# 1879615351/Go-RIO

Hardware: AMD Instinct MI355X
Metric: APD-GICP GN iters/sec on 16k-pt scans + GP-preint windows/sec (higher is better)
Workload: dtype f32 search / f64 accumulate; 1 GPU; C4: 64 scan pairs 16384x16384 + 64 GP windows 1 s @ 200 Hz per GPU, k-NN covariances + 20 fixed GN iterations per pair; pairs_per_gpu=64, target_points=16384, optimizer=GN (convergence test disabled), search=pruned, parallelism=batch shard x1 (no collective)

## Files before the change

### go-rio_amd/csrc/ugpm_api.hip

```cpp
#include <hip/hip_runtime.h>

#include <algorithm>
#include <cmath>
#include <cstdlib>
#include <chrono>
#include <cstdio>
#include <cstring>
#include <limits>
#include <memory>
#include <string>
#include <atomic>
#include <vector>

#include "../../include/gorio_ugpm.h"
#include "ugpm_kernels.hip"
#include "ugpm_lpm_out.hip"
#include "ugpm_chunks.h"

using namespace gorio;

namespace {

#ifndef GORIO_EVAL_SPLIT
#define GORIO_EVAL_SPLIT 12
// ... 8 lines not shown
  int device = -1;
  hipStream_t stream = nullptr;
  hipStream_t stream2 = nullptr;
  hipEvent_t ev_jac = nullptr, ev_corr = nullptr, ev_up = nullptr;
  struct Group { hipStream_t s = nullptr, s2 = nullptr; hipEvent_t ev_jac = nullptr, ev_corr = nullptr, ev_done = nullptr, ev_tab = nullptr; };
  std::vector<Group> groups;
  double* ws = nullptr;
  size_t ws_cap = 0;
  UgpmWin* d_wins = nullptr;
  int wins_cap = 0;
  int* d_ints = nullptr;
  int lm_budget[2] = {0, 0};
  double* d_diag = nullptr;
  double* pin_in = nullptr;
  size_t pin_in_cap = 0;
  double* lpm_ws = nullptr;
  size_t lpm_ws_cap = 0;
  int* lpm_ints = nullptr;
  size_t lpm_ints_cap = 0;
  ug::LpmOutWin* d_lpm_wins = nullptr;
  int lpm_wins_cap = 0;
  std::vector<std::pair<hipEvent_t, hipEvent_t>> ev;
  std::vector<int> ev_stage;
};
thread_local Ctx g_ctx;
std::atomic<int> g_speculative_rot{1};

int ufail(int code, const std::string& msg) {
  g_err = msg;
  return code;
}

#define UHIP(expr)                                                                                              \
  do {                                                                                                          \
    hipError_t e_ = (expr);                                                                                     \
    if (e_ != hipSuccess) return ufail(GORIO_UGPM_ERR_NO_DEVICE, std::string(#expr) + ": " + hipGetErrorString(e_)); \
  } while (0)

struct HostWin {
  int g0 = 0, G = 0, v0 = 0, V = 0, S = 0;
  double state_freq = 0;
// ... 126 lines not shown
void gorio_ugpm_default_window(gorio_ugpm_window* w) {
  if (!w) return;
  std::memset(w, 0, sizeof(*w));
  w->type = GORIO_UGPM_TYPE_UGPM;
  w->min_freq = 500;
  w->quantum = -1;
  w->state_freq = 50.0;
  w->correlate = 1;
  w->overlap = 8;
  w->vel_bias_std = 0.3;
  w->gyr_bias_std = 0.03;
}

const char* gorio_ugpm_last_error(void) { return g_err.c_str(); }

void gorio_ugpm_debug_set_schedule(int speculative_rot) { g_speculative_rot.store(speculative_rot ? 1 : 0); }

int gorio_ugpm_get_stage_times(double seconds[8], int counts[8]) {
  for (int i = 0; i < 8; ++i) {
    if (seconds) seconds[i] = g_stage_s[i];
    if (counts) counts[i] = g_stage_n[i];
  }
  return 0;
}

static int preint_batch_flat(const gorio_ugpm_window* windows, int n_windows, gorio_ugpm_meas* out, gorio_ugpm_diag* diag, int device) {
  if (!windows || n_windows <= 0 || !out) return ufail(GORIO_UGPM_ERR_INVALID, "gorio_ugpm_preint_batch: bad arguments");
  int ndev = 0;
  if (hipGetDeviceCount(&ndev) != hipSuccess || ndev <= 0) return ufail(GORIO_UGPM_ERR_NO_DEVICE, "no usable HIP device (no CPU fallback exists)");
  if (device < 0 || device >= ndev) return ufail(GORIO_UGPM_ERR_INVALID, "bad device ordinal");
  UHIP(hipSetDevice(device));
  Ctx& c = g_ctx;
  if (c.device != device) {
    for (size_t g = 1; g < c.groups.size(); ++g) {
      hipStreamDestroy(c.groups[g].s); hipStreamDestroy(c.groups[g].s2);
      hipEventDestroy(c.groups[g].ev_jac); hipEventDestroy(c.groups[g].ev_corr);
    }
    for (auto& g : c.groups) { hipEventDestroy(g.ev_done); hipEventDestroy(g.ev_tab); }
    if (c.ev_up) hipEventDestroy(c.ev_up);
    if (c.stream) hipStreamDestroy(c.stream);
    if (c.stream2) hipStreamDestroy(c.stream2);
    if (c.ev_jac) hipEventDestroy(c.ev_jac);
    if (c.ev_corr) hipEventDestroy(c.ev_corr);
    hipFree(c.ws); hipFree(c.d_wins); hipFree(c.d_ints); hipFree(c.d_diag); hipFree(c.lpm_ws); hipFree(c.lpm_ints); hipFree(c.d_lpm_wins);
    if (c.pin_in) hipHostFree(c.pin_in);
    c = Ctx();
    c.device = device;
    bool made = false;
    if (!made) {
      int lo = 0, hi = 0;
      if (hipDeviceGetStreamPriorityRange(&lo, &hi) == hipSuccess && hipStreamCreateWithPriority(&c.stream, hipStreamNonBlocking, hi) == hipSuccess) made = true;
    }
    if (!made) UHIP(hipStreamCreateWithFlags(&c.stream, hipStreamNonBlocking));
    UHIP(hipStreamCreateWithFlags(&c.stream2, hipStreamNonBlocking));
    UHIP(hipEventCreateWithFlags(&c.ev_jac, hipEventDisableTiming));
    UHIP(hipEventCreateWithFlags(&c.ev_corr, hipEventDisableTiming));
    UHIP(hipFuncSetAttribute(reinterpret_cast<const void*>(&ug::corr_diag_kernel), hipFuncAttributeMaxDynamicSharedMemorySize, 140 * 1024));
    UHIP(hipFuncSetAttribute(reinterpret_cast<const void*>(&ug::infer_kernel), hipFuncAttributeMaxDynamicSharedMemorySize, 17 * (6 * 160 + 16) * 8) );
    {
      const void* fns[] = {reinterpret_cast<const void*>(&ug::ata_kernel<4, 16, kAtaTilesCorr>), reinterpret_cast<const void*>(&ug::ata_kernel<8, 16, kAtaTilesCorr>),
// ... 316 lines not shown
        ug::cross_kernel<<<dim3(12, r.nw, (std::max(max_G, max_V) + ug::kCrossRows - 1) / ug::kCrossRows), 256, sizeof(double) * ug::kCrossRows * (((max_S + 31) / 32) * 32 + 4), r.s>>>(dw_);
      }
      UHIP(hipEventRecord(r.ev_tab, r.s));
      UHIP(hipStreamWaitEvent(r.s2, r.ev_tab, 0));
      {
        Stage st(c, 2, r.s2);
        ug::corr_jac_kernel<<<dim3(ug::kCorrJacParts, r.nw), 256, 0, r.s2>>>(dw_);
        UHIP(hipEventRecord(r.ev_jac, r.s2));
        launch_ata(r, 2);
        ug::corr_factor_kernel<<<r.nw, 512, 0, r.s2>>>(dw_);
        ug::corr_diag_kernel<<<dim3((6 * max_S + 15) / 16, r.nw), 256, sizeof(double) * 17 * (6 * max_S + 16), r.s2>>>(dw_);
      }
      UHIP(hipEventRecord(r.ev_corr, r.s2));
    }
    std::vector<int> flags(kWinInts * (size_t)nw);
    const bool speculative = g_speculative_rot.load() != 0;
    for (int problem = 0; problem < 2; ++problem) {
      std::vector<std::unique_ptr<Stage>> st_lm;
      for (Run& r : runs) {
        const UgpmWin* dw_ = c.d_wins + r.g0;
        st_lm.emplace_back(new Stage(c, 3, r.s));
        ug::lm_begin_kernel<<<r.nw, 256, 0, r.s>>>(dw_, problem);
        if (problem == 0) ug::rot_eval_kernel<<<dim3(r.nw, kEvalSplit), 256, 0, r.s>>>(dw_, 2);
        else ug::vel_eval_kernel<<<dim3(r.nw, kEvalSplit), 256, 0, r.s>>>(dw_, 2);
        launch_ata(r, problem);
        r.active = true;
      }
      for (int it = 0; it <= 51; ++it) {
        bool any = false;
        for (Run& r : runs) {
          if (!r.active) continue;
          any = true;
          const UgpmWin* dw_ = c.d_wins + r.g0;
          ug::lm_step_kernel<<<dim3(r.nw, problem == 1 ? kVelBlocks : 1), 512, 0, r.s>>>(dw_);
          if (problem == 0 && speculative) {
            ug::rot_eval_kernel<<<dim3(r.nw, kEvalSplit), 256, 0, r.s>>>(dw_, 3);
            launch_ata(r, problem, 1);
            continue;
          }
          if (problem == 0) ug::rot_eval_kernel<<<dim3(r.nw, kEvalSplit), 256, 0, r.s>>>(dw_, 0);
          else ug::vel_eval_kernel<<<dim3(r.nw, kEvalSplit), 256, 0, r.s>>>(dw_, 0);
          if (problem == 0) {
            ug::rot_eval_kernel<<<dim3(r.nw, kEvalSplit), 256, 0, r.s>>>(dw_, 1);
// ... 45 lines not shown
    }
    for (Run& r : runs) {
      const UgpmWin* dw_ = c.d_wins + r.g0;
      UHIP(hipStreamWaitEvent(r.s, r.ev_corr, 0));
      {
        Stage st(c, 4, r.s);
        ug::finish_kernel<<<r.nw, 256, 0, r.s>>>(dw_);
        ug::infer_kernel<<<dim3(std::max(1, max_infer), r.nw), 256, sizeof(double) * 17 * (6 * max_S + 16), r.s>>>(dw_);
      }
      UHIP(hipEventRecord(r.ev_done, r.s));
    }
    for (size_t g = 1; g < runs.size(); ++g) UHIP(hipStreamWaitEvent(c.stream, runs[g].ev_done, 0));
    UHIP(hipGetLastError());
  }
  tt3 = tnow();
  std::vector<int> fin(kWinInts * (size_t)nw);
  std::vector<double> dg(4 * (size_t)nw);
  UHIP(hipMemcpyAsync(fin.data(), c.d_ints, sizeof(int) * fin.size(), hipMemcpyDeviceToHost, c.stream));
  UHIP(hipMemcpyAsync(dg.data(), c.d_diag, sizeof(double) * dg.size(), hipMemcpyDeviceToHost, c.stream));
  if (total_out) UHIP(hipMemcpyAsync(reinterpret_cast<double*>(out), out_region, sizeof(double) * total_out, hipMemcpyDeviceToHost, c.stream));
  UHIP(hipStreamSynchronize(c.stream));
  for (size_t q = 0; q < c.ev.size(); ++q) {
    float ms = 0.f;
    if (hipEventSynchronize(c.ev[q].second) == hipSuccess && hipEventElapsedTime(&ms, c.ev[q].first, c.ev[q].second) == hipSuccess) {
      g_stage_s[c.ev_stage[q]] += ms * 1e-3;
      g_stage_n[c.ev_stage[q]] += 1;
    }
    hipEventDestroy(c.ev[q].first);
    hipEventDestroy(c.ev[q].second);
  }
  c.ev.clear();
  c.ev_stage.clear();
  for (int i = 0; i < nw; ++i) {
    if (hw[i].status != 0) {
// ... 137 lines not shown
```

### go-rio_amd/csrc/ugpm_kernels.hip

```cpp
#include <hip/hip_runtime.h>
#include <math.h>

#include "ugpm_device.h"

namespace gorio {
namespace ug {

__device__ __forceinline__ UgpmWin load_win(const UgpmWin* __restrict__ wins, int i) {
  UgpmWin w;
  __builtin_memcpy(&w, (const __attribute__((address_space(4))) void*)(wins + i), sizeof(UgpmWin));
  return w;
}


#ifndef GORIO_UGPM_XCD
#define GORIO_UGPM_XCD 1
#endif
struct WinPart {
  int win, part, z;
};
__device__ __forceinline__ WinPart xcd_win_part() {
  WinPart r{(int)blockIdx.y, (int)blockIdx.x, (int)blockIdx.z};
#if GORIO_UGPM_XCD
  if (gridDim.y >= 16u && (gridDim.y & 7u) == 0u) {
// ... 1009 lines not shown
  }
}


__device__ __forceinline__ void small_gemm_tn_sym(const double* __restrict__ B, double* __restrict__ C, int S) {
  const int lane = threadIdx.x & 63, wave = threadIdx.x >> 6, nwave = (int)(blockDim.x >> 6);
  const int lr = lane & 15, lk = lane >> 4;
  const int T = (S + 15) / 16;
  for (int q = wave; q < T * (T + 1) / 2; q += nwave) {
    int tr = (int)((sqrtf(8.0f * (float)q + 1.0f) - 1.0f) * 0.5f);
    while (tr * (tr + 1) / 2 > q) --tr;
    while ((tr + 1) * (tr + 2) / 2 <= q) ++tr;
    const int tc = q - tr * (tr + 1) / 2;
    const int i = tr * 16 + lr, j = tc * 16 + lr;
    f64x4 acc = f64x4{0.0, 0.0, 0.0, 0.0};
#pragma unroll 4
    for (int k0 = tr * 16; k0 < S; k0 += 4) {
      const int k = k0 + lk;
      const double av = (k < S && i < S) ? B[(size_t)k * S + i] : 0.0;
      const double bv = (k < S && j < S) ? B[(size_t)k * S + j] : 0.0;
      acc = __builtin_amdgcn_mfma_f64_16x16x4f64(av, bv, acc, 0, 0, 0);
    }
#pragma unroll
    for (int rg = 0; rg < 4; ++rg) {
      const int r = tr * 16 + lk + 4 * rg, c = tc * 16 + lr;
      if (r < S && c < S) {
        C[(size_t)r * S + c] = acc[rg];
        C[(size_t)c * S + r] = acc[rg];
      }
    }
  }
}
__device__ __forceinline__ void small_gemm_nn(const double* __restrict__ A, const double* __restrict__ B, double* __restrict__ C, int S) {
  const int lane = threadIdx.x & 63, wave = threadIdx.x >> 6, nwave = (int)(blockDim.x >> 6);
  const int lr = lane & 15, lk = lane >> 4;
  const int T = (S + 15) / 16;
  for (int q = wave; q < T * T; q += nwave) {
    const int ti = q / T, tj = q - ti * T;
    const int i = ti * 16 + lr, j = tj * 16 + lr;
    f64x4 acc = f64x4{0.0, 0.0, 0.0, 0.0};
#pragma unroll 4
    for (int k0 = 0; k0 < S; k0 += 4) {
      const int k = k0 + lk;
      const double av = (k < S && i < S) ? A[(size_t)i * S + k] : 0.0;
      const double bv = (k < S && j < S) ? B[(size_t)k * S + j] : 0.0;
      acc = __builtin_amdgcn_mfma_f64_16x16x4f64(av, bv, acc, 0, 0, 0);
    }
#pragma unroll
    for (int rg = 0; rg < 4; ++rg) {
      const int r = ti * 16 + lk + 4 * rg, c = tj * 16 + lr;
      if (r < S && c < S) C[(size_t)r * S + c] = acc[rg];
    }
  }
}

__global__ __launch_bounds__(256) __attribute__((amdgpu_waves_per_eu(2, 2))) void gram_kernel(const UgpmWin* __restrict__ wins) {
// ... 88 lines not shown
  for (int r = wave; r < kCrossRows; r += 4) {
    const int n = row0 + r;
    for (int k = lane; k < LDK; k += 64) {
      double v = 0.0;
      if (n < N && k < S) v = integral ? se_kint(w.start_t, tt[n], w.state_t[k], l2, sf2) : se_k(tt[n], w.state_t[k], l2, sf2);
      ks[(size_t)r * LDK + k] = v;
    }
  }
  __syncthreads();
  const int lr = lane & 15, lk = lane >> 4;
  const int TJ = (S + 15) / 16;
  for (int q = wave; q < 2 * TJ; q += 4) {
    const int ti = q / TJ, tj = q - ti * TJ;
    const int j = tj * 16 + lr;
    f64x4 acc = f64x4{0.0, 0.0, 0.0, 0.0};
#pragma unroll 4
    for (int k0 = 0; k0 < S; k0 += 4) {
      const int k = k0 + lk;
      const double av = ks[(size_t)(ti * 16 + lr) * LDK + k];
      const double bv = (k < S && j < S) ? Ki[(size_t)k * S + j] : 0.0;
      acc = __builtin_amdgcn_mfma_f64_16x16x4f64(av, bv, acc, 0, 0, 0);
    }
#pragma unroll
    for (int rg = 0; rg < 4; ++rg) {
      const int n = row0 + ti * 16 + lk + 4 * rg;
      if (n < N && j < S) out[(size_t)n * S + j] = acc[rg];
    }
  }
}


// ... 73 lines not shown
  }
#pragma unroll
  for (int off = 32; off > 0; off >>= 1)
#pragma unroll
    for (int q = 0; q < 3; ++q) t[q] += __shfl_xor(t[q], off, 64);
#pragma unroll
  for (int q = 0; q < 3; ++q) out[q] = t[q];
}

__device__ __forceinline__ void lm_step_bookkeeping(const UgpmWin& w) {
  w.lmi[3] = 0;
  w.lmi[8] = 0;
  w.lmi[0] += 1;
}

__device__ int lm_decide_block(const UgpmWin& w, int m, int n, bool commit, double* sred ) {
  const int nblk = w.lmi[7] == 1 ? kVelBlocks : 1;
  bool step_ok = true;
  double mcc = 0.0, sn2 = 0.0;
  for (int q = 0; q < nblk; ++q) {
    step_ok = step_ok && w.lmi[9 + q] != 0;
    mcc += w.lmc[8 + q];
    sn2 += w.lmc[11 + q];
  }
  if (!(mcc > 0.0)) step_ok = false;
  const double sn = sqrt(sn2);
  if (!step_ok) {
    if (commit && threadIdx.x == 0) {
      w.lmc[2] = w.lmc[2] / w.lmc[3];
      w.lmc[3] *= 2.0;
// ... 14 lines not shown
  else if (fabs(cost_change) <= 1e-10 * cost) verdict = -1;
  else {
    rho = cost_change / mcc;
    verdict = rho > 1e-3 ? 1 : 0;
  }
  __syncthreads();
  if (commit) {
    if (threadIdx.x == 0) {
      w.lmc[1] = cost_new;
      if (verdict < 0) {
        w.lmi[1] = 1;
        w.lmi[5] = verdict == -2 ? 2 : 1;
      } else if (verdict == 1) {
        w.lmi[6] += 1;
        w.lmi[3] = 1;
        w.lmc[2] = fmin(1e16, w.lmc[2] / fmax(1.0 / 3.0, 1.0 - pow(2.0 * rho - 1.0, 3)));
        w.lmc[3] = 2.0;
        w.lmi[2] = 0;
      } else {
        w.lmc[2] = w.lmc[2] / w.lmc[3];
        w.lmc[3] *= 2.0;
        w.lmi[2] = 1;
      }
    }
    if (verdict == 1)
      for (int j = threadIdx.x; j < n; j += blockDim.x) w.lmv[5 * (size_t)n + j] = w.lmv[6 * (size_t)n + j];
  }
  return verdict < 0 ? -1 : verdict;
}

__device__ void gpnorm_rows(const UgpmWin& w, int ch, const double* __restrict__ s, double* __restrict__ res, double* __restrict__ J, int ldj, int col0, bool writeJ) {
  const int S = w.S;
  const double* KK = w.KKinv + (size_t)ch * S * S;
  const double* wt = w.wgp + (size_t)ch * S;
  if ((int)blockIdx.y != ch % (int)gridDim.y) return;
  for (int i = threadIdx.x; i < S; i += blockDim.x) res[i] = (row_dot(KK + (size_t)i * S, s, S) - s[i]) * wt[i];
  if (writeJ)
    for (int q = threadIdx.x; q < S * S; q += blockDim.x) {
      const int i = q / S, j = q % S;
      J[(size_t)i * ldj + col0 + j] = (KK[(size_t)j * S + i] - (i == j ? 1.0 : 0.0)) * wt[i];
    }
}

__global__ __launch_bounds__(256) void rot_eval_kernel(const UgpmWin* __restrict__ wins, int mode) {
  const UgpmWin w = load_win(wins, blockIdx.x);
  if (*w.status != 0 || w.lmi[1]) return;
  const int S = w.S, G = w.G, n = 3 * S;
  __shared__ double sred[8];
  if ((mode == 0 || mode == 3) && blockIdx.y == 0 && threadIdx.x == 0) lm_step_bookkeeping(w);
  if (mode == 1) {
    if (lm_decide_block(w, 3 * S + 3 * G, n, blockIdx.y == 0, sred) != 1) return;
  }
  const double* x = mode == 2 ? w.lmv + 5 * (size_t)n : w.lmv + 6 * (size_t)n;
  double* res = (mode == 0 || mode == 3) ? w.res_new : w.res;
  double* J = w.Jrot;
  const int i_lo = (int)(((long)G * blockIdx.y) / gridDim.y), i_hi = (int)(((long)G * (blockIdx.y + 1)) / gridDim.y);
// ... 52 lines not shown
        const double* k1 = w.KsKinv + ((size_t)c * G + i) * S;
        for (int j = lane; j < S; j += 64) row[c * S + j] = f0 * k0[j] + f1 * k1[j];
      }
    }
  }
}

__device__ __forceinline__ V3 vel_rot_vec(const UgpmWin& w, int i) {
  const int S = w.S, V = w.V;
  double rot[3];
  for (int c = 0; c < 3; ++c) rot[c] = row_dot(w.KgyrIntKinv + ((size_t)c * V + i) * S, w.s_dr + (size_t)c * S, S);
  const double dtm = w.vel_t[i] - w.start_t;
  return v3(rot[0] + dtm * w.hyper[3], rot[1] + dtm * w.hyper[7], rot[2] + dtm * w.hyper[11]);
}

__global__ __launch_bounds__(256) void vel_eval_kernel(const UgpmWin* __restrict__ wins, int mode) {
  const UgpmWin w = load_win(wins, blockIdx.x);
  if (*w.status != 0 || w.lmi[1]) return;
  if (mode == 1 && !w.lmi[3]) return;
  if (mode == 0 && blockIdx.y == 0 && threadIdx.x == 0) lm_step_bookkeeping(w);
  const int S = w.S, V = w.V, n = 3 * S;
  const double* x = mode == 0 ? w.lmv + 6 * (size_t)n : w.lmv + 5 * (size_t)n;
  double* res = mode == 0 ? w.res_new : w.res;
  double* J = w.Jvel;
  const int i_lo = (int)(((long)V * blockIdx.y) / gridDim.y), i_hi = (int)(((long)V * (blockIdx.y + 1)) / gridDim.y);
  if (mode == 2) {
    for (int c = 0; c < 3; ++c)
      if ((int)blockIdx.y == (3 + c) % (int)gridDim.y)
        for (size_t q = threadIdx.x; q < (size_t)S * n; q += blockDim.x) J[((size_t)3 * V + (size_t)c * S) * n + q] = 0.0;
    for (size_t q = threadIdx.x; q < (size_t)(i_hi - i_lo) * 3 * n; q += blockDim.x) J[(size_t)i_lo * 3 * n + q] = 0.0;
  }
  __syncthreads();
  for (int c = 0; c < 3; ++c) gpnorm_rows(w, 3 + c, x + (size_t)c * S, res + 3 * V + (size_t)c * S, J + ((size_t)3 * V + (size_t)c * S) * n, n, c * S, mode == 2);
  const double wgt = sqrt(1.0 / w.vel_var);
  __shared__ double sdot[256][6];
  for (int ib = i_lo; ib < i_hi; ib += 256) {
    const int cnt = min(256, i_hi - ib);
    for (int q = (int)(threadIdx.x >> 6); q < cnt; q += (int)(blockDim.x >> 6)) {
      const int i = ib + q;
      if (mode == 0) {
        double d3[3];
        wave_row_dots3(w.KvelKinv + (size_t)i * S, (size_t)V * S, x, S, d3);
        if ((threadIdx.x & 63) == 0) {
#pragma unroll
          for (int q2 = 0; q2 < 3; ++q2) sdot[q][3 + q2] = d3[q2];
        }
      } else {
        double d[6];
        wave_row_dots6(w.KgyrIntKinv + (size_t)i * S, (size_t)V * S, w.s_dr, w.KvelKinv + (size_t)i * S, (size_t)V * S, x, S, d);
        if ((threadIdx.x & 63) == 0) {
#pragma unroll
          for (int q2 = 0; q2 < 6; ++q2) sdot[q][q2] = d[q2];
        }
      }
    }
    __syncthreads();
    for (int q = threadIdx.x; q < cnt; q += blockDim.x) {
      const int i = ib + q;
      M3 RT;
      if (mode == 0) {
        RT = loadM(w.sample_tmp + (size_t)i * 24);
      } else {
        const double dtm = w.vel_t[i] - w.start_t;
        const V3 rv = v3(sdot[q][0] + dtm * w.hyper[3], sdot[q][1] + dtm * w.hyper[7], sdot[q][2] + dtm * w.hyper[11]);
        RT = expMap(v3(-rv.x, -rv.y, -rv.z));
      }
      const V3 vv = v3(sdot[q][3] + w.hyper[15], sdot[q][4] + w.hyper[19], sdot[q][5] + w.hyper[23]);
      const V3 t = mvec(RT, vv);
      double* r = res + 3 * i;
      r[0] = (t.x - (w.vel[i] - w.vel_bias[0])) * wgt;
      r[1] = (t.y - (w.vel[V + i] - w.vel_bias[1])) * wgt;
      r[2] = (t.z - (w.vel[2 * V + i] - w.vel_bias[2])) * wgt;
      if (mode != 0) storeM(w.sample_tmp + (size_t)i * 24, RT);
    }
    __syncthreads();
  }
  if (mode == 0) return;
  __syncthreads();
  {
    const int wave = threadIdx.x >> 6, lane = threadIdx.x & 63, nwave = (int)(blockDim.x >> 6);
    for (int rr = wave; rr < (i_hi - i_lo) * 3; rr += nwave) {
      const int i = i_lo + rr / 3, a = rr % 3;
      double* row = J + (size_t)(3 * i + a) * n;
      for (int c = 0; c < 3; ++c) {
        const double f = wgt * w.sample_tmp[(size_t)i * 24 + a * 3 + c];
        const double* k0 = w.KvelKinv + ((size_t)c * V + i) * S;
        for (int j = lane; j < S; j += 64) row[c * S + j] = f * k0[j];
      }
    }
  }
}
// ... 249 lines not shown
    }
    if (g != nullptr) {
      __syncthreads();
      if (gpart < gparts) ata_lds[gpart * gcolw + (int)threadIdx.x % gcolw] = gcol ? gacc : 0.0;
      __syncthreads();
      if (tid < gj1 - gj0) {
        double v = 0.0;
        for (int q = 0; q < gparts; ++q) v += ata_lds[q * gcolw + tid];
        g[gj0 + tid] = v;
      }
    }
  }
  CHOL_T(7);
}

__global__ __launch_bounds__(256) void lm_relinearize_linear_kernel(const UgpmWin* __restrict__ wins) {
  const UgpmWin w = load_win(wins, blockIdx.x);
  if (*w.status != 0 || w.lmi[1]) return;
  const int n = 3 * w.S, m = 3 * w.V + 3 * w.S;
  const int j0 = blockIdx.y * 64;
  if (j0 >= n) return;
  __shared__ double sred[8];
  if (lm_decide_block(w, m, n, blockIdx.y == 0, sred) != 1) return;
  const double* J = w.Jvel;
  const double* rn = w.res_new;
  __shared__ double sg[4][64];
  if (blockIdx.y == 0)
    for (int k = threadIdx.x; k < m; k += blockDim.x) w.res[k] = rn[k];
  const int slice = threadIdx.x >> 6, lane = threadIdx.x & 63;
  const int j = j0 + lane;
  double acc[4] = {0.0, 0.0, 0.0, 0.0};
  if (j < n) {
    int k = slice;
    for (; k + 12 < m; k += 16) {
#pragma unroll
      for (int u = 0; u < 4; ++u) acc[u] += J[(size_t)(k + 4 * u) * n + j] * rn[k + 4 * u];
    }
    for (; k < m; k += 4) acc[0] += J[(size_t)k * n + j] * rn[k];
  }
  sg[slice][lane] = (acc[0] + acc[1]) + (acc[2] + acc[3]);
  __syncthreads();
  if (slice == 0 && j < n) w.lmv[j] = (sg[0][lane] + sg[1][lane]) + (sg[2][lane] + sg[3][lane]);
}


__global__ __launch_bounds__(256) void lm_begin_kernel(const UgpmWin* __restrict__ wins, int problem) {
  const UgpmWin w = load_win(wins, blockIdx.x);
  if (*w.status != 0) return;
  const int n = 3 * w.S;
  const double* src = problem == 0 ? w.s_dr : w.s_vel;
  for (int j = threadIdx.x; j < n; j += blockDim.x) w.lmv[5 * (size_t)n + j] = src[j];
  if (threadIdx.x == 0) {
    for (int q = 0; q < 16; ++q) w.lmi[q] = 0;
    w.lmi[3] = 1;
    w.lmi[7] = problem;
    w.lmi[8] = 1;
    w.lmc[2] = 1e4;
    w.lmc[3] = 2.0;
  }
}

__global__ __launch_bounds__(512) void lm_step_kernel(const UgpmWin* __restrict__ wins) {
  const UgpmWin w = load_win(wins, blockIdx.x);
  if (*w.status != 0 || w.lmi[1]) return;
  const int n = 3 * w.S;
  const int problem = w.lmi[7];
  const int m = problem == 0 ? 3 * w.S + 3 * w.G : 3 * w.V + 3 * w.S;
  const int nblk = (int)gridDim.y, blk = (int)blockIdx.y;
  const int j0 = (int)((long)n * blk / nblk), j1 = (int)((long)n * (blk + 1) / nblk), ns = j1 - j0;
  double* g = w.lmv;
  double* scale = w.lmv + (size_t)n;
  double* diag = w.lmv + 2 * (size_t)n;
  double* step = w.lmv + 3 * (size_t)n;
  double* delta = w.lmv + 4 * (size_t)n;
  double* x = w.lmv + 5 * (size_t)n;
  double* xn = w.lmv + 6 * (size_t)n;
  __shared__ double sred[8];
  __shared__ int sflag;
  __shared__ CholLds chol;
  if (w.lmi[3]) {
    double c = 0.0;
    for (int k = threadIdx.x; k < m; k += blockDim.x) c += w.res[k] * w.res[k];
    c = 0.5 * block_sum(c, sred);
    double gm = 0.0, xn2 = 0.0;
    for (int j = threadIdx.x; j < n; j += blockDim.x) {
      gm = fmax(gm, fabs(g[j]));
      xn2 += x[j] * x[j];
    }
    gm = block_max(gm, sred);
    xn2 = block_sum(xn2, sred);
    if (w.lmi[8])
      for (int j = j0 + (int)threadIdx.x; j < j1; j += blockDim.x) scale[j] = 1.0 / (1.0 + sqrt(w.JtJ[(size_t)j * n + j]));
    __syncthreads();
    if (threadIdx.x == 0) {
      w.lmc[0] = c;
      w.lmc[4] = sqrt(xn2);
      if (w.lmi[8]) w.lmc[7] = c;
      if (gm <= 1e-10) {
        w.lmi[1] = 1;
        w.lmi[5] = 3;
      }
    }
    if (gm <= 1e-10) return;
  }
  if (w.lmi[0] >= 50) {
    if (threadIdx.x == 0) { w.lmi[1] = 1; w.lmi[5] = 4; }
    return;
  }
  const double radius = w.lmc[2];
  if (radius < 1e-32) {
    if (threadIdx.x == 0) { w.lmi[1] = 1; w.lmi[5] = 5; }
    return;
  }
  if (!w.lmi[2])
    for (int j = j0 + (int)threadIdx.x; j < j1; j += blockDim.x) diag[j] = fmin(fmax(w.JtJ[(size_t)j * n + j] * scale[j] * scale[j], 1e-6), 1e32);
  __syncthreads();
  double* L = w.lhs + (size_t)j0 * n + j0;
  __shared__ double xs[kCholMaxN / 2];
  const bool fused = ns < 384 && ns <= (int)blockDim.x && ns <= kCholMaxN / 2;
  for (int i = threadIdx.x >> 6; i < ns; i += (int)(blockDim.x >> 6)) {
    const double si = scale[j0 + i];
    for (int j = threadIdx.x & 63; j <= i; j += 64)
      L[(size_t)i * n + j] = w.JtJ[(size_t)(j0 + i) * n + j0 + j] * si * scale[j0 + j] + (i == j ? diag[j0 + i] / radius : 0.0);
  }
  double* rhs = w.lmv + 7 * (size_t)n + j0;
  for (int j = threadIdx.x; j < ns; j += blockDim.x) {
    step[j0 + j] = g[j0 + j] * scale[j0 + j];
    if (fused) rhs[j] = g[j0 + j] * scale[j0 + j];
  }
  __syncthreads();
  bool valid = block_cholesky(L, ns, n, chol, &sflag, fused ? rhs : nullptr);
  if (valid) {
    if (fused) {
      for (int j = threadIdx.x; j < ns; j += blockDim.x) xs[j] = rhs[j];
      __syncthreads();
      block_backward(L, ns, n, xs, chol);
      for (int j = threadIdx.x; j < ns; j += blockDim.x) step[j0 + j] = xs[j];
    } else {
      double* xp = &chol.P[0][0];
      for (int j = threadIdx.x; j < ns; j += blockDim.x) xp[j] = step[j0 + j];
      __syncthreads();
      if (threadIdx.x < 64) {
        wave_forward<1>(L, ns, n, xp, 1, 0);
        wave_backward(L, ns, n, xp);
      }
      __syncthreads();
// ... 16 lines not shown
      const double hi = 0.5 * delta[i];
      for (int j = j0 + (int)(threadIdx.x & 63); j < j1; j += 64) acc += hi * w.JtJ[(size_t)i * n + j] * delta[j];
    }
    for (int i = j0 + (int)threadIdx.x; i < j1; i += blockDim.x) {
      acc += delta[i] * g[i];
      sn2 += delta[i] * delta[i];
      xn[i] = x[i] + delta[i];
    }
    mcc = -block_sum(acc, sred);
    sn2 = block_sum(sn2, sred);
  }
  if (threadIdx.x == 0) {
    w.lmi[9 + blk] = valid ? 1 : 0;
    w.lmc[8 + blk] = mcc;
    w.lmc[11 + blk] = sn2;
  }
}


__global__ __launch_bounds__(256) void lm_end_kernel(const UgpmWin* __restrict__ wins, int problem, double* __restrict__ diag_out ) {
  const UgpmWin w = load_win(wins, blockIdx.x);
  if (*w.status != 0) return;
  const int n = 3 * w.S;
  double* dst = problem == 0 ? w.s_dr : w.s_vel;
  for (int j = threadIdx.x; j < n; j += blockDim.x) dst[j] = w.lmv[5 * (size_t)n + j];
  if (threadIdx.x == 0) {
    diag_out[blockIdx.x * 4 + problem * 2 + 0] = (double)w.lmi[0];
    diag_out[blockIdx.x * 4 + problem * 2 + 1] = w.lmc[0];
  }
}
// ... 273 lines not shown
```

### go-rio_amd/ugpm.py

```python
import ctypes as C

import numpy as np

from .apd import GorioError, load_library

LPM, UGPM = 0, 1
REC = 83

UGPM_SYMBOLS = ["gorio_ugpm_default_window", "gorio_ugpm_preint_batch", "gorio_ugpm_last_error", "gorio_ugpm_get_stage_times", "gorio_ugpm_debug_set_schedule",
                "gorio_ugpm_combine_preints"]


class UgpmWindow(C.Structure):

    _fields_ = [
        ("gyr_t", C.c_void_p), ("gyr", C.c_void_p), ("n_gyr", C.c_int),
        ("vel_t", C.c_void_p), ("vel", C.c_void_p), ("n_vel", C.c_int),
        ("gyr_var", C.c_double), ("vel_var", C.c_double), ("start_t", C.c_double),
        ("infer_t", C.c_void_p), ("n_infer", C.c_int), ("type", C.c_int),
        ("min_freq", C.c_double), ("quantum", C.c_double), ("state_freq", C.c_double),
        ("correlate", C.c_int), ("overlap", C.c_int),
        ("gyr_bias", C.c_double * 3), ("vel_bias", C.c_double * 3),
        ("vel_bias_std", C.c_double), ("gyr_bias_std", C.c_double),
        ("group_sizes", C.c_void_p), ("n_groups", C.c_int),
# ... 91 lines not shown
    return np.concatenate([np.asarray(m["delta_R"], np.float64).ravel(), np.asarray(m["delta_p"], np.float64), [m["dt"], m["dt_sq_half"]],
                           np.asarray(m["cov"], np.float64).ravel(), np.asarray(m["d_delta_R_d_bw"], np.float64).ravel(), np.asarray(m["d_delta_R_d_t"], np.float64),
                           np.asarray(m["d_delta_p_d_bw"], np.float64).ravel(), np.asarray(m["d_delta_p_d_bv"], np.float64).ravel(), np.asarray(m["d_delta_p_d_t"], np.float64)])


def ugpm_combine_preints(prev, cur):
    lib = load_library()
    a, b, out = np.ascontiguousarray(pack(prev)), np.ascontiguousarray(pack(cur)), np.zeros(REC)
    lib.gorio_ugpm_combine_preints.argtypes = [C.c_void_p, C.c_void_p, C.c_void_p]
    rc = lib.gorio_ugpm_combine_preints(C.c_void_p(_dp(a)), C.c_void_p(_dp(b)), C.c_void_p(_dp(out)))
    if rc < 0:
        raise GorioError(rc, lib.gorio_ugpm_last_error().decode())
    return unpack(out)


def ugpm_debug_set_schedule(speculative_rot=True):
    lib = load_library()
    lib.gorio_ugpm_debug_set_schedule.argtypes = [C.c_int]
    lib.gorio_ugpm_debug_set_schedule.restype = None
    lib.gorio_ugpm_debug_set_schedule(1 if speculative_rot else 0)


def ugpm_stage_times():
    lib = load_library()
    s = (C.c_double * 8)()
    c = (C.c_int * 8)()
    lib.gorio_ugpm_get_stage_times(s, c)
    return list(s), list(c)


class PreintOption:

    def __init__(self, min_freq=500.0, type=UGPM, quantum=-1.0, state_freq=50.0, correlate=True):
        self.min_freq, self.type, self.quantum, self.state_freq, self.correlate = min_freq, type, quantum, state_freq, correlate

# ... 59 lines not shown
```

### include/gorio_ugpm.h

```cpp
#ifndef GORIO_UGPM_H
#define GORIO_UGPM_H

#ifdef __cplusplus
extern "C" {
#endif

typedef enum {
  GORIO_UGPM_OK = 0,
  GORIO_UGPM_ERR_INVALID = -1,
  GORIO_UGPM_ERR_NO_DEVICE = -2,
  GORIO_UGPM_ERR_RANGE = -3,
  GORIO_UGPM_ERR_ARGUMENT = -4,
  GORIO_UGPM_ERR_UNSUPPORTED = -5,
  GORIO_UGPM_ERR_NUMERIC = -6
} gorio_ugpm_status;

typedef enum { GORIO_UGPM_TYPE_LPM = 0, GORIO_UGPM_TYPE_UGPM = 1 } gorio_ugpm_type;

typedef struct {
  const double* gyr_t;
  const double* gyr;
  int n_gyr;
  const double* vel_t;
  const double* vel;
// ... 40 lines not shown
  double cost_rot;
  double cost_vel;
  double state_freq;
} gorio_ugpm_diag;

void gorio_ugpm_default_window(gorio_ugpm_window* w);

int gorio_ugpm_preint_batch(const gorio_ugpm_window* windows, int n_windows, gorio_ugpm_meas* out, gorio_ugpm_diag* diag, int device);

int gorio_ugpm_combine_preints(const gorio_ugpm_meas* prev, const gorio_ugpm_meas* cur, gorio_ugpm_meas* out);

const char* gorio_ugpm_last_error(void);

int gorio_ugpm_get_stage_times(double seconds[8], int counts[8]);

void gorio_ugpm_debug_set_schedule(int speculative_rot);

#ifdef __cplusplus
}
#endif
#endif
```

Measured before the change: 164,500 linearisations/s.

## Fuse velocity LM solve into a single persistent per-window kernel launch

Adds vel_fit_kernel, which runs the whole velocity-problem Levenberg-Marquardt loop (step, residual evaluation, decision, gradient update) inside one launch per run. It replaces up to 52 host-driven passes of separate kernel launches and is the default schedule. The step, residual and gradient code is factored into shared device helpers. Output readback moves to a reusable pinned host buffer, and several GEMM loops change from unroll 4 to unroll 1, presumably to relieve register pressure. The risk is that one block per window serialises work that was previously split across kVelBlocks blocks, and that aliasing shared memory between the Cholesky panel and the scratch arrays needs careful synchronisation.

Result: slower. 142,300 linearisations/s (-13.5%).

```diff
diff --git a/go-rio_amd/csrc/ugpm_api.hip b/go-rio_amd/csrc/ugpm_api.hip
--- a/go-rio_amd/csrc/ugpm_api.hip
+++ b/go-rio_amd/csrc/ugpm_api.hip
@@ -46,6 +46,8 @@
   double* d_diag = nullptr;
   double* pin_in = nullptr;
   size_t pin_in_cap = 0;
+  char* pin_out = nullptr;
+  size_t pin_out_cap = 0;
   double* lpm_ws = nullptr;
   size_t lpm_ws_cap = 0;
   int* lpm_ints = nullptr;
@@ -56,7 +58,8 @@
   std::vector<int> ev_stage;
 };
 thread_local Ctx g_ctx;
-std::atomic<int> g_speculative_rot{1};
+std::atomic<int> g_schedule{1};
+constexpr int kLmMaxPasses = 52;
 
 int ufail(int code, const std::string& msg) {
   g_err = msg;
@@ -213,7 +216,7 @@
 
 const char* gorio_ugpm_last_error(void) { return g_err.c_str(); }
 
-void gorio_ugpm_debug_set_schedule(int speculative_rot) { g_speculative_rot.store(speculative_rot ? 1 : 0); }
+void gorio_ugpm_debug_set_schedule(int schedule) { g_schedule.store(schedule & 3); }
 
 int gorio_ugpm_get_stage_times(double seconds[8], int counts[8]) {
   for (int i = 0; i < 8; ++i) {
@@ -243,6 +246,7 @@
     if (c.ev_corr) hipEventDestroy(c.ev_corr);
     hipFree(c.ws); hipFree(c.d_wins); hipFree(c.d_ints); hipFree(c.d_diag); hipFree(c.lpm_ws); hipFree(c.lpm_ints); hipFree(c.d_lpm_wins);
     if (c.pin_in) hipHostFree(c.pin_in);
+    if (c.pin_out) hipHostFree(c.pin_out);
     c = Ctx();
     c.device = device;
     bool made = false;
@@ -589,7 +593,9 @@
       UHIP(hipEventRecord(r.ev_corr, r.s2));
     }
     std::vector<int> flags(kWinInts * (size_t)nw);
-    const bool speculative = g_speculative_rot.load() != 0;
+    const int schedule = g_schedule.load();
+    const bool speculative = (schedule & 1) != 0;
+    const bool fused_vel = (schedule & 2) == 0;
     for (int problem = 0; problem < 2; ++problem) {
       std::vector<std::unique_ptr<Stage>> st_lm;
       for (Run& r : runs) {
@@ -601,7 +607,23 @@
         launch_ata(r, problem);
         r.active = true;
       }
-      for (int it = 0; it <= 51; ++it) {
+      if (problem == 1 && fused_vel) {
+        for (size_t g = 0; g < runs.size(); ++g) {
+          ug::vel_fit_kernel<<<runs[g].nw, 512, 0, runs[g].s>>>(c.d_wins + runs[g].g0, kLmMaxPasses, c.d_diag + 4 * (size_t)runs[g].g0);
+          st_lm[g].reset();
+        }
+        if (lmtrace) {
+          double lc[16];
+          int li[16];
+          UHIP(hipStreamSynchronize(runs[0].s));
+          UHIP(hipMemcpy(lc, dw[0].lmc, sizeof(lc), hipMemcpyDeviceToHost));
+          UHIP(hipMemcpy(li, dw[0].lmi, sizeof(li), hipMemcpyDeviceToHost));
+          std::fprintf(stderr, "[ugpm lm] problem 1 (one launch): iter %d done %d term %d succ %d cost %.17g cost_new %.17g radius %.6g x_norm %.17g initial %.17g\n",
+                       li[0], li[1], li[5], li[6], lc[0], lc[1], lc[2], lc[4], lc[7]);
+        }
+        continue;
+      }
+      for (int it = 0; it < kLmMaxPasses; ++it) {
         bool any = false;
         for (Run& r : runs) {
           if (!r.active) continue;
@@ -677,10 +699,18 @@
     UHIP(hipGetLastError());
   }
   tt3 = tnow();
-  std::vector<int> fin(kWinInts * (size_t)nw);
-  std::vector<double> dg(4 * (size_t)nw);
-  UHIP(hipMemcpyAsync(fin.data(), c.d_ints, sizeof(int) * fin.size(), hipMemcpyDeviceToHost, c.stream));
-  UHIP(hipMemcpyAsync(dg.data(), c.d_diag, sizeof(double) * dg.size(), hipMemcpyDeviceToHost, c.stream));
+  const size_t dg_bytes = sizeof(double) * 4 * (size_t)nw, fin_bytes = sizeof(int) * kWinInts * (size_t)nw;
+  if (dg_bytes + fin_bytes > c.pin_out_cap) {
+    if (c.pin_out) hipHostFree(c.pin_out);
+    c.pin_out = nullptr;
+    c.pin_out_cap = 0;
+    UHIP(hipHostMalloc(reinterpret_cast<void**>(&c.pin_out), 2 * (dg_bytes + fin_bytes), hipHostMallocDefault));
+    c.pin_out_cap = 2 * (dg_bytes + fin_bytes);
+  }
+  const double* const dg = reinterpret_cast<const double*>(c.pin_out);
+  const int* const fin = reinterpret_cast<const int*>(c.pin_out + dg_bytes);
+  UHIP(hipMemcpyAsync(c.pin_out + dg_bytes, c.d_ints, fin_bytes, hipMemcpyDeviceToHost, c.stream));
+  UHIP(hipMemcpyAsync(c.pin_out, c.d_diag, dg_bytes, hipMemcpyDeviceToHost, c.stream));
   if (total_out) UHIP(hipMemcpyAsync(reinterpret_cast<double*>(out), out_region, sizeof(double) * total_out, hipMemcpyDeviceToHost, c.stream));
   UHIP(hipStreamSynchronize(c.stream));
   for (size_t q = 0; q < c.ev.size(); ++q) {
diff --git a/go-rio_amd/csrc/ugpm_kernels.hip b/go-rio_amd/csrc/ugpm_kernels.hip
--- a/go-rio_amd/csrc/ugpm_kernels.hip
+++ b/go-rio_amd/csrc/ugpm_kernels.hip
@@ -1047,7 +1047,7 @@
     const int tc = q - tr * (tr + 1) / 2;
     const int i = tr * 16 + lr, j = tc * 16 + lr;
     f64x4 acc = f64x4{0.0, 0.0, 0.0, 0.0};
-#pragma unroll 4
+#pragma unroll 1
     for (int k0 = tr * 16; k0 < S; k0 += 4) {
       const int k = k0 + lk;
       const double av = (k < S && i < S) ? B[(size_t)k * S + i] : 0.0;
@@ -1072,7 +1072,7 @@
     const int ti = q / T, tj = q - ti * T;
     const int i = ti * 16 + lr, j = tj * 16 + lr;
     f64x4 acc = f64x4{0.0, 0.0, 0.0, 0.0};
-#pragma unroll 4
+#pragma unroll 1
     for (int k0 = 0; k0 < S; k0 += 4) {
       const int k = k0 + lk;
       const double av = (k < S && i < S) ? A[(size_t)i * S + k] : 0.0;
@@ -1191,7 +1191,7 @@
     const int ti = q / TJ, tj = q - ti * TJ;
     const int j = tj * 16 + lr;
     f64x4 acc = f64x4{0.0, 0.0, 0.0, 0.0};
-#pragma unroll 4
+#pragma unroll 1
     for (int k0 = 0; k0 < S; k0 += 4) {
       const int k = k0 + lk;
       const double av = ks[(size_t)(ti * 16 + lr) * LDK + k];
@@ -1295,6 +1295,8 @@
   w.lmi[0] += 1;
 }
 
+__device__ __noinline__ double lm_cube(double v) { return pow(v, 3); }
+
 __device__ int lm_decide_block(const UgpmWin& w, int m, int n, bool commit, double* sred ) {
   const int nblk = w.lmi[7] == 1 ? kVelBlocks : 1;
   bool step_ok = true;
@@ -1339,7 +1341,7 @@
       } else if (verdict == 1) {
         w.lmi[6] += 1;
         w.lmi[3] = 1;
-        w.lmc[2] = fmin(1e16, w.lmc[2] / fmax(1.0 / 3.0, 1.0 - pow(2.0 * rho - 1.0, 3)));
+        w.lmc[2] = fmin(1e16, w.lmc[2] / fmax(1.0 / 3.0, 1.0 - lm_cube(2.0 * rho - 1.0)));
         w.lmc[3] = 2.0;
         w.lmi[2] = 0;
       } else {
@@ -1354,17 +1356,20 @@
   return verdict < 0 ? -1 : verdict;
 }
 
-__device__ void gpnorm_rows(const UgpmWin& w, int ch, const double* __restrict__ s, double* __restrict__ res, double* __restrict__ J, int ldj, int col0, bool writeJ) {
+__device__ void gpnorm_rows_block(const UgpmWin& w, int ch, const double* __restrict__ s, double* __restrict__ res, double* __restrict__ J, int ldj, int col0, bool writeJ) {
   const int S = w.S;
   const double* KK = w.KKinv + (size_t)ch * S * S;
   const double* wt = w.wgp + (size_t)ch * S;
-  if ((int)blockIdx.y != ch % (int)gridDim.y) return;
   for (int i = threadIdx.x; i < S; i += blockDim.x) res[i] = (row_dot(KK + (size_t)i * S, s, S) - s[i]) * wt[i];
   if (writeJ)
     for (int q = threadIdx.x; q < S * S; q += blockDim.x) {
       const int i = q / S, j = q % S;
       J[(size_t)i * ldj + col0 + j] = (KK[(size_t)j * S + i] - (i == j ? 1.0 : 0.0)) * wt[i];
     }
+}
+__device__ void gpnorm_rows(const UgpmWin& w, int ch, const double* __restrict__ s, double* __restrict__ res, double* __restrict__ J, int ldj, int col0, bool writeJ) {
+  if ((int)blockIdx.y != ch % (int)gridDim.y) return;
+  gpnorm_rows_block(w, ch, s, res, J, ldj, col0, writeJ);
 }
 
 __global__ __launch_bounds__(256) void rot_eval_kernel(const UgpmWin* __restrict__ wins, int mode) {
@@ -1447,6 +1452,52 @@
   return v3(rot[0] + dtm * w.hyper[3], rot[1] + dtm * w.hyper[7], rot[2] + dtm * w.hyper[11]);
 }
 
+__device__ __forceinline__ void vel_residual_rows(const UgpmWin& w, int mode, const double* __restrict__ x, double* __restrict__ res, int i_lo, int i_hi, double (*sdot)[6]) {
+  const int S = w.S, V = w.V;
+  const double wgt = sqrt(1.0 / w.vel_var);
+  for (int ib = i_lo; ib < i_hi; ib += 256) {
+    const int cnt = min(256, i_hi - ib);
+    for (int q = (int)(threadIdx.x >> 6); q < cnt; q += (int)(blockDim.x >> 6)) {
+      const int i = ib + q;
+      if (mode == 0) {
+        double d3[3];
+        wave_row_dots3(w.KvelKinv + (size_t)i * S, (size_t)V * S, x, S, d3);
+        if ((threadIdx.x & 63) == 0) {
+#pragma unroll
+          for (int q2 = 0; q2 < 3; ++q2) sdot[q][3 + q2] = d3[q2];
+        }
+      } else {
+        double d[6];
+        wave_row_dots6(w.KgyrIntKinv + (size_t)i * S, (size_t)V * S, w.s_dr, w.KvelKinv + (size_t)i * S, (size_t)V * S, x, S, d);
+        if ((threadIdx.x & 63) == 0) {
+#pragma unroll
+          for (int q2 = 0; q2 < 6; ++q2) sdot[q][q2] = d[q2];
+        }
+      }
+    }
+    __syncthreads();
+    for (int q = threadIdx.x; q < cnt; q += blockDim.x) {
+      const int i = ib + q;
+      M3 RT;
+      if (mode == 0) {
+        RT = loadM(w.sample_tmp + (size_t)i * 24);
+      } else {
+        const double dtm = w.vel_t[i] - w.start_t;
+        const V3 rv = v3(sdot[q][0] + dtm * w.hyper[3], sdot[q][1] + dtm * w.hyper[7], sdot[q][2] + dtm * w.hyper[11]);
+        RT = expMap(v3(-rv.x, -rv.y, -rv.z));
+      }
+      const V3 vv = v3(sdot[q][3] + w.hyper[15], sdot[q][4] + w.hyper[19], sdot[q][5] + w.hyper[23]);
+      const V3 t = mvec(RT, vv);
+      double* r = res + 3 * i;
+      r[0] = (t.x - (w.vel[i] - w.vel_bias[0])) * wgt;
+      r[1] = (t.y - (w.vel[V + i] - w.vel_bias[1])) * wgt;
+      r[2] = (t.z - (w.vel[2 * V + i] - w.vel_bias[2])) * wgt;
+      if (mode != 0) storeM(w.sample_tmp + (size_t)i * 24, RT);
+    }
+    __syncthreads();
+  }
+}
+
 __global__ __launch_bounds__(256) void vel_eval_kernel(const UgpmWin* __restrict__ wins, int mode) {
   const UgpmWin w = load_win(wins, blockIdx.x);
   if (*w.status != 0 || w.lmi[1]) return;
@@ -1467,47 +1518,7 @@
   for (int c = 0; c < 3; ++c) gpnorm_rows(w, 3 + c, x + (size_t)c * S, res + 3 * V + (size_t)c * S, J + ((size_t)3 * V + (size_t)c * S) * n, n, c * S, mode == 2);
   const double wgt = sqrt(1.0 / w.vel_var);
   __shared__ double sdot[256][6];
-  for (int ib = i_lo; ib < i_hi; ib += 256) {
-    const int cnt = min(256, i_hi - ib);
-    for (int q = (int)(threadIdx.x >> 6); q < cnt; q += (int)(blockDim.x >> 6)) {
-      const int i = ib + q;
-      if (mode == 0) {
-        double d3[3];
-        wave_row_dots3(w.KvelKinv + (size_t)i * S, (size_t)V * S, x, S, d3);
-        if ((threadIdx.x & 63) == 0) {
-#pragma unroll
-          for (int q2 = 0; q2 < 3; ++q2) sdot[q][3 + q2] = d3[q2];
-        }
-      } else {
-        double d[6];
-        wave_row_dots6(w.KgyrIntKinv + (size_t)i * S, (size_t)V * S, w.s_dr, w.KvelKinv + (size_t)i * S, (size_t)V * S, x, S, d);
-        if ((threadIdx.x & 63) == 0) {
-#pragma unroll
-          for (int q2 = 0; q2 < 6; ++q2) sdot[q][q2] = d[q2];
-        }
-      }
-    }
-    __syncthreads();
-    for (int q = threadIdx.x; q < cnt; q += blockDim.x) {
-      const int i = ib + q;
-      M3 RT;
-      if (mode == 0) {
-        RT = loadM(w.sample_tmp + (size_t)i * 24);
-      } else {
-        const double dtm = w.vel_t[i] - w.start_t;
-        const V3 rv = v3(sdot[q][0] + dtm * w.hyper[3], sdot[q][1] + dtm * w.hyper[7], sdot[q][2] + dtm * w.hyper[11]);
-        RT = expMap(v3(-rv.x, -rv.y, -rv.z));
-      }
-      const V3 vv = v3(sdot[q][3] + w.hyper[15], sdot[q][4] + w.hyper[19], sdot[q][5] + w.hyper[23]);
-      const V3 t = mvec(RT, vv);
-      double* r = res + 3 * i;
-      r[0] = (t.x - (w.vel[i] - w.vel_bias[0])) * wgt;
-      r[1] = (t.y - (w.vel[V + i] - w.vel_bias[1])) * wgt;
-      r[2] = (t.z - (w.vel[2 * V + i] - w.vel_bias[2])) * wgt;
-      if (mode != 0) storeM(w.sample_tmp + (size_t)i * 24, RT);
-    }
-    __syncthreads();
-  }
+  vel_residual_rows(w, mode, x, res, i_lo, i_hi, sdot);
   if (mode == 0) return;
   __syncthreads();
   {
@@ -1787,6 +1798,20 @@
   CHOL_T(7);
 }
 
+__device__ __forceinline__ double linear_gradient_slice(const double* __restrict__ J, const double* __restrict__ rn, int n, int m, int j, int slice) {
+  double acc[4] = {0.0, 0.0, 0.0, 0.0};
+  if (j < n) {
+    int k = slice;
+#pragma unroll 2
+    for (; k + 12 < m; k += 16) {
+#pragma unroll
+      for (int u = 0; u < 4; ++u) acc[u] += J[(size_t)(k + 4 * u) * n + j] * rn[k + 4 * u];
+    }
+    for (; k < m; k += 4) acc[0] += J[(size_t)k * n + j] * rn[k];
+  }
+  return (acc[0] + acc[1]) + (acc[2] + acc[3]);
+}
+
 __global__ __launch_bounds__(256) void lm_relinearize_linear_kernel(const UgpmWin* __restrict__ wins) {
   const UgpmWin w = load_win(wins, blockIdx.x);
   if (*w.status != 0 || w.lmi[1]) return;
@@ -1802,16 +1827,7 @@
     for (int k = threadIdx.x; k < m; k += blockDim.x) w.res[k] = rn[k];
   const int slice = threadIdx.x >> 6, lane = threadIdx.x & 63;
   const int j = j0 + lane;
-  double acc[4] = {0.0, 0.0, 0.0, 0.0};
-  if (j < n) {
-    int k = slice;
-    for (; k + 12 < m; k += 16) {
-#pragma unroll
-      for (int u = 0; u < 4; ++u) acc[u] += J[(size_t)(k + 4 * u) * n + j] * rn[k + 4 * u];
-    }
-    for (; k < m; k += 4) acc[0] += J[(size_t)k * n + j] * rn[k];
-  }
-  sg[slice][lane] = (acc[0] + acc[1]) + (acc[2] + acc[3]);
+  sg[slice][lane] = linear_gradient_slice(J, rn, n, m, j, slice);
   __syncthreads();
   if (slice == 0 && j < n) w.lmv[j] = (sg[0][lane] + sg[1][lane]) + (sg[2][lane] + sg[3][lane]);
 }
@@ -1833,24 +1849,18 @@
   }
 }
 
-__global__ __launch_bounds__(512) void lm_step_kernel(const UgpmWin* __restrict__ wins) {
-  const UgpmWin w = load_win(wins, blockIdx.x);
-  if (*w.status != 0 || w.lmi[1]) return;
-  const int n = 3 * w.S;
-  const int problem = w.lmi[7];
-  const int m = problem == 0 ? 3 * w.S + 3 * w.G : 3 * w.V + 3 * w.S;
-  const int nblk = (int)gridDim.y, blk = (int)blockIdx.y;
-  const int j0 = (int)((long)n * blk / nblk), j1 = (int)((long)n * (blk + 1) / nblk), ns = j1 - j0;
+struct LmStepLds {
+  double sred[8];
+  int sflag;
+  CholLds chol;
+  double xs[kCholMaxN / 2];
+};
+
+__device__ __forceinline__ bool lm_step_head(const UgpmWin& w, int n, int m, int j0, int j1, LmStepLds& sh) {
   double* g = w.lmv;
   double* scale = w.lmv + (size_t)n;
-  double* diag = w.lmv + 2 * (size_t)n;
-  double* step = w.lmv + 3 * (size_t)n;
-  double* delta = w.lmv + 4 * (size_t)n;
   double* x = w.lmv + 5 * (size_t)n;
-  double* xn = w.lmv + 6 * (size_t)n;
-  __shared__ double sred[8];
-  __shared__ int sflag;
-  __shared__ CholLds chol;
+  double* sred = sh.sred;
   if (w.lmi[3]) {
     double c = 0.0;
     for (int k = threadIdx.x; k < m; k += blockDim.x) c += w.res[k] * w.res[k];
@@ -1874,22 +1884,36 @@
         w.lmi[5] = 3;
       }
     }
-    if (gm <= 1e-10) return;
+    if (gm <= 1e-10) return false;
   }
   if (w.lmi[0] >= 50) {
     if (threadIdx.x == 0) { w.lmi[1] = 1; w.lmi[5] = 4; }
-    return;
-  }
+    return false;
+  }
+  if (w.lmc[2] < 1e-32) {
+    if (threadIdx.x == 0) { w.lmi[1] = 1; w.lmi[5] = 5; }
+    return false;
+  }
+  return true;
+}
+
+__device__ __forceinline__ void lm_step_block(const UgpmWin& w, int n, int j0, int j1, int blk, LmStepLds& sh) {
+  const int ns = j1 - j0;
+  double* g = w.lmv;
+  double* scale = w.lmv + (size_t)n;
+  double* diag = w.lmv + 2 * (size_t)n;
+  double* step = w.lmv + 3 * (size_t)n;
+  double* delta = w.lmv + 4 * (size_t)n;
+  double* x = w.lmv + 5 * (size_t)n;
+  double* xn = w.lmv + 6 * (size_t)n;
+  double* sred = sh.sred;
+  CholLds& chol = sh.chol;
+  double* xs = sh.xs;
   const double radius = w.lmc[2];
-  if (radius < 1e-32) {
-    if (threadIdx.x == 0) { w.lmi[1] = 1; w.lmi[5] = 5; }
-    return;
-  }
   if (!w.lmi[2])
     for (int j = j0 + (int)threadIdx.x; j < j1; j += blockDim.x) diag[j] = fmin(fmax(w.JtJ[(size_t)j * n + j] * scale[j] * scale[j], 1e-6), 1e32);
   __syncthreads();
   double* L = w.lhs + (size_t)j0 * n + j0;
-  __shared__ double xs[kCholMaxN / 2];
   const bool fused = ns < 384 && ns <= (int)blockDim.x && ns <= kCholMaxN / 2;
   for (int i = threadIdx.x >> 6; i < ns; i += (int)(blockDim.x >> 6)) {
     const double si = scale[j0 + i];
@@ -1902,7 +1926,7 @@
     if (fused) rhs[j] = g[j0 + j] * scale[j0 + j];
   }
   __syncthreads();
-  bool valid = block_cholesky(L, ns, n, chol, &sflag, fused ? rhs : nullptr);
+  bool valid = block_cholesky(L, ns, n, chol, &sh.sflag, fused ? rhs : nullptr);
   if (valid) {
     if (fused) {
       for (int j = threadIdx.x; j < ns; j += blockDim.x) xs[j] = rhs[j];
@@ -1949,6 +1973,89 @@
     w.lmi[9 + blk] = valid ? 1 : 0;
     w.lmc[8 + blk] = mcc;
     w.lmc[11 + blk] = sn2;
+  }
+}
+
+__global__ __launch_bounds__(512) void lm_step_kernel(const UgpmWin* __restrict__ wins) {
+  const UgpmWin w = load_win(wins, blockIdx.x);
+  if (*w.status != 0 || w.lmi[1]) return;
+  const int n = 3 * w.S;
+  const int problem = w.lmi[7];
+  const int m = problem == 0 ? 3 * w.S + 3 * w.G : 3 * w.V + 3 * w.S;
+  const int nblk = (int)gridDim.y, blk = (int)blockIdx.y;
+  const int j0 = (int)((long)n * blk / nblk), j1 = (int)((long)n * (blk + 1) / nblk);
+  __shared__ LmStepLds sh;
+  if (!lm_step_head(w, n, m, j0, j1, sh)) return;
+  lm_step_block(w, n, j0, j1, blk, sh);
+}
+
+__global__ __launch_bounds__(512) void vel_fit_kernel(const UgpmWin* __restrict__ wins, int max_passes, double* __restrict__ diag_out ) {
+  __shared__ LmStepLds sh;
+  double (*sdot)[6] = reinterpret_cast<double (*)[6]>(&sh.chol.P[0][0]);
+  double (*sg)[4][64] = reinterpret_cast<double (*)[4][64]>(&sh.chol.P[0][0]);
+  static_assert(sizeof(sh.chol.P) >= 256 * 6 * sizeof(double) && sizeof(sh.chol.P) >= 2 * 4 * 64 * sizeof(double), "panel buffer too small for the aliases");
+  auto win = [&]() {
+    const UgpmWin* p = wins;
+    asm volatile("" : "+s"(p));
+    return load_win(p, blockIdx.x);
+  };
+  {
+    const UgpmWin w = win();
+    if (*w.status != 0) return;
+  }
+#pragma unroll 1
+  for (int pass = 0; pass < max_passes; ++pass) {
+    bool go;
+    {
+      const UgpmWin w = win();
+      const int n = 3 * w.S;
+      go = !w.lmi[1];
+      if (go) go = lm_step_head(w, n, 3 * w.V + n, 0, n, sh);
+    }
+    __syncthreads();
+    if (!go) break;
+#pragma unroll 1
+    for (int blk = 0; blk < kVelBlocks; ++blk) {
+      const UgpmWin w = win();
+      const int n = 3 * w.S;
+      lm_step_block(w, n, (int)((long)n * blk / kVelBlocks), (int)((long)n * (blk + 1) / kVelBlocks), blk, sh);
+      __syncthreads();
+    }
+    {
+      const UgpmWin w = win();
+      const int S = w.S, V = w.V, n = 3 * S;
+      const double* xn = w.lmv + 6 * (size_t)n;
+      if (threadIdx.x == 0) lm_step_bookkeeping(w);
+      for (int c = 0; c < 3; ++c) gpnorm_rows_block(w, 3 + c, xn + (size_t)c * S, w.res_new + 3 * V + (size_t)c * S, nullptr, n, c * S, false);
+      vel_residual_rows(w, 0, xn, w.res_new, 0, V, sdot);
+    }
+    __syncthreads();
+    {
+      const UgpmWin w = win();
+      const int n = 3 * w.S, m = 3 * w.V + n;
+      if (lm_decide_block(w, m, n, true, sh.sred) == 1) {
+        for (int k = threadIdx.x; k < m; k += blockDim.x) w.res[k] = w.res_new[k];
+        const int team = threadIdx.x >> 8, slice = (threadIdx.x >> 6) & 3, lane = threadIdx.x & 63;
+        for (int c0 = 0; c0 * 64 < n; c0 += 2) {
+          const int j = (c0 + team) * 64 + lane;
+          __syncthreads();
+          sg[team][slice][lane] = linear_gradient_slice(w.Jvel, w.res_new, n, m, j, slice);
+          __syncthreads();
+          if (slice == 0 && j < n) w.lmv[j] = (sg[team][0][lane] + sg[team][1][lane]) + (sg[team][2][lane] + sg[team][3][lane]);
+        }
+      }
+    }
+    __syncthreads();
+  }
+  __syncthreads();
+  {
+    const UgpmWin w = win();
+    const int n = 3 * w.S;
+    for (int j = threadIdx.x; j < n; j += blockDim.x) w.s_vel[j] = w.lmv[5 * (size_t)n + j];
+    if (threadIdx.x == 0) {
+      diag_out[blockIdx.x * 4 + 2] = (double)w.lmi[0];
+      diag_out[blockIdx.x * 4 + 3] = w.lmc[0];
+    }
   }
 }
 
diff --git a/go-rio_amd/ugpm.py b/go-rio_amd/ugpm.py
--- a/go-rio_amd/ugpm.py
+++ b/go-rio_amd/ugpm.py
@@ -129,11 +129,11 @@
     return unpack(out)
 
 
-def ugpm_debug_set_schedule(speculative_rot=True):
+def ugpm_debug_set_schedule(speculative_rot=True, per_iteration_vel=False):
     lib = load_library()
     lib.gorio_ugpm_debug_set_schedule.argtypes = [C.c_int]
     lib.gorio_ugpm_debug_set_schedule.restype = None
-    lib.gorio_ugpm_debug_set_schedule(1 if speculative_rot else 0)
+    lib.gorio_ugpm_debug_set_schedule((1 if speculative_rot else 0) | (2 if per_iteration_vel else 0))
 
 
 def ugpm_stage_times():
diff --git a/include/gorio_ugpm.h b/include/gorio_ugpm.h
--- a/include/gorio_ugpm.h
+++ b/include/gorio_ugpm.h
@@ -78,7 +78,7 @@
 
 int gorio_ugpm_get_stage_times(double seconds[8], int counts[8]);
 
-void gorio_ugpm_debug_set_schedule(int speculative_rot);
+void gorio_ugpm_debug_set_schedule(int schedule);
 
 #ifdef __cplusplus
 }
```
